# inai17ibar/video-diffusion-pipeline-parallel

Measured on AMD Instinct MI355X. Metric: steady-state videos/sec (whole node), SVD 14f x 25step, higher is better.
Workload: dtype f16

## Files before the change

video-diffusion-pipeline-parallel_amd/csrc/attention_long.hip:

```cpp
#include "common.h"

namespace {

typedef unsigned u32x4 __attribute__((ext_vector_type(4)));
typedef unsigned u32x2 __attribute__((ext_vector_type(2)));

__device__ __forceinline__ float fast_exp2(float x) { return __builtin_amdgcn_exp2f(x); }

constexpr unsigned LONG_BAIL_MIN = 64, LONG_BAIL_MAX = 512;

template <int QB>
__global__ __launch_bounds__(256, 1) void attn_long_kernel(
    const f16 *__restrict__ q, const f16 *__restrict__ k, const f16 *__restrict__ v, f16 *__restrict__ o,
    int64_t ldq, int64_t ldk, int64_t ldv, int64_t ldo, int seq, int heads, float scale_log2e,
    unsigned *__restrict__ flags) {
  constexpr int KV = 64;
  constexpr int K_BYTES = KV * 128, STAGE = 2 * K_BYTES, RING = 3;
  constexpr int OWN = 2 * QB;
  constexpr int WARM = OWN + 1;
  __shared__ __attribute__((aligned(16))) char smem[RING * STAGE];

  const int tid = threadIdx.x, lane = tid & 63;
  const int wave = __builtin_amdgcn_readfirstlane(tid >> 6);
  const int bh = blockIdx.y;
  {
    unsigned *const flagged_waves = flags + (int64_t)gridDim.x * gridDim.y;
    if (tid == 0) *(volatile unsigned *)smem = __hip_atomic_load(flagged_waves, __ATOMIC_RELAXED, __HIP_MEMORY_SCOPE_AGENT);
    __syncthreads();
    const unsigned seen = *(volatile unsigned *)smem;
    __syncthreads();
    const unsigned total_waves = gridDim.x * gridDim.y * 4u;
    const unsigned frac = total_waves / 16u;
    const unsigned bail = frac < LONG_BAIL_MIN ? LONG_BAIL_MIN : (frac > LONG_BAIL_MAX ? LONG_BAIL_MAX : frac);
    if (seen >= bail) {
      if (tid == 0) flags[(int64_t)bh * gridDim.x + blockIdx.x] = 1u;
      return;
    }
  }
  const int b = bh / heads, hd = bh - b * heads;
  const int r = lane & 31, h = lane >> 5;
  const int64_t row0 = (int64_t)b * seq;
  const int q0 = blockIdx.x * (128 * QB) + wave * (32 * QB);

  f16x8 qf[QB][4];
#pragma unroll
  for (int qb = 0; qb < QB; ++qb) {
    const f16 *qp = q + (row0 + q0 + qb * 32 + r) * ldq + hd * 64 + 8 * h;
#pragma unroll
    for (int s = 0; s < 4; ++s) {
      const f16x8 raw = *(const f16x8 *)(qp + 16 * s);
#pragma unroll
      for (int e = 0; e < 8; ++e) qf[qb][s][e] = (f16)((float)raw[e] * scale_log2e);
    }
  }

  const int lrow = lane >> 3, lchunk = lane & 7;
  unsigned kofl[2], vofl[2];
#pragma unroll
  for (int i = 0; i < 2; ++i) {
    const int row = wave * 16 + i * 8 + lrow;
    kofl[i] = (unsigned)((row * ldk + ((lchunk ^ ((row >> 1) & 7)) << 3)) * 2);
    vofl[i] = (unsigned)((row * ldv + ((lchunk ^ (((row >> 1) & 1) << 2)) << 3)) * 2);
  }
  const int64_t kstep = (int64_t)KV * ldk * 2, vstep = (int64_t)KV * ldv * 2;

  int koff[2];
#pragma unroll
  for (int kt = 0; kt < 2; ++kt) koff[kt] = (kt * 32 + r) * 128;
  int kswz = (r >> 1) & 7, hq = h;
  const int g = lane >> 4, i16 = lane & 15, q_ = i16 >> 2, pp = i16 & 3;
  const int vrow_l = 4 * (g >> 1) + q_;
  const int vchunk_l = 2 * (g & 1) + (pp >> 1);
  const int vswz = (q_ >> 1) << 2;
  const int vbyte_l = (pp & 1) * 8;
  int vlane0 = vrow_l * 128 + ((vchunk_l ^ vswz) << 4) + vbyte_l;
  int vlane1 = vrow_l * 128 + (((4 + vchunk_l) ^ vswz) << 4) + vbyte_l;

  f16x8 lsel;
  {
    const int m16 = lane & 15, kb4 = lane >> 4;
    const bool one = ((m16 & 7) == 0 && (kb4 & 1) == 0) || ((m16 & 7) == 4 && (kb4 & 1) == 1);
#pragma unroll
    for (int e = 0; e < 8; ++e) lsel[e] = one ? (f16)1.f : (f16)0.f;
  }

  f32x16 oacc[QB][2], negm[QB];
  f32x4 lacc[QB];
  float m_run[QB];
#pragma unroll
  for (int qb = 0; qb < QB; ++qb) {
    m_run[qb] = 0.f;
    lacc[qb] = (f32x4){0.f, 0.f, 0.f, 0.f};
#pragma unroll
    for (int e = 0; e < 16; ++e) { oacc[qb][0][e] = 0.f; oacc[qb][1][e] = 0.f; negm[qb][e] = 0.f; }
  }
  const int ntiles = seq / KV;

  const int own0 = blockIdx.x * OWN;
  const char *kbase = (const char *)(k + row0 * ldk + hd * 64);
  const char *vbase = (const char *)(v + row0 * ldv + hd * 64);
  auto stage = [&](int i, int buf) {
    const int tl = i < OWN ? own0 + i : (i - OWN < own0 ? i - OWN : i);
    const char *kb = kbase + tl * kstep, *vb = vbase + tl * vstep;
    char *sk = smem + buf * STAGE;
    char *sv = sk + K_BYTES;
#pragma unroll
    for (int j = 0; j < 2; ++j) {
      glds16(kb + kofl[j], sk + (wave * 16 + j * 8) * 128);
      glds16(vb + vofl[j], sv + (wave * 16 + j * 8) * 128);
    }
  };
  stage(0, 0);
  stage(1, 1);
  asm volatile("s_waitcnt vmcnt(4)" ::: "memory");
  __builtin_amdgcn_s_barrier();

  auto qk = [&](int qb, const char *sk, f32x16 (&sacc)[2]) {
    f16x8 kf[2][4];
#pragma unroll
    for (int kt = 0; kt < 2; ++kt)
#pragma unroll
      for (int s = 0; s < 4; ++s) kf[kt][s] = *(const f16x8 *)(sk + koff[kt] + (((2 * s + hq) ^ kswz) << 4));
#pragma unroll
    for (int kt = 0; kt < 2; ++kt)
#pragma unroll
      for (int s = 0; s < 4; ++s)
        sacc[kt] = __builtin_amdgcn_mfma_f32_32x32x16_f16(kf[kt][s], qf[qb][s], s == 0 ? negm[qb] : sacc[kt], 0, 0, 0);
  };
  auto pv = [&](int qb, const u32x4 (&pw)[2][2], const u32x2 (&vr)[2][8]) {
#pragma unroll
    for (int dt = 0; dt < 2; ++dt)
#pragma unroll
      for (int kt = 0; kt < 2; ++kt)
#pragma unroll
        for (int s = 0; s < 2; ++s) {
          const u32x4 vw = {vr[dt][4 * kt + 2 * s][0], vr[dt][4 * kt + 2 * s][1], vr[dt][4 * kt + 2 * s + 1][0],
                            vr[dt][4 * kt + 2 * s + 1][1]};
          oacc[qb][dt] = __builtin_amdgcn_mfma_f32_32x32x16_f16(__builtin_bit_cast(f16x8, vw),
                                                               __builtin_bit_cast(f16x8, pw[kt][s]), oacc[qb][dt], 0, 0, 0);
          if (dt == 0)
            lacc[qb] = __builtin_amdgcn_mfma_f32_16x16x32_f16(lsel, __builtin_bit_cast(f16x8, pw[kt][s]), lacc[qb], 0, 0, 0);
        }
  };

  auto warm_tile = [&](int i, int buf) {
    if (i + 2 < ntiles) stage(i + 2, buf >= 1 ? buf - 1 : RING - 1);
    const char *sk = smem + buf * STAGE;
    const char *sv = sk + K_BYTES;

    f32x16 sacc[2][2];
    u32x4 pw[2][2][2];
    qk(0, sk, sacc[0]);
    u32x2 vr[2][8];
    {
      const unsigned va[2] = {(unsigned)(uintptr_t)(const __attribute__((address_space(3))) char *)(sv + vlane0),
                              (unsigned)(uintptr_t)(const __attribute__((address_space(3))) char *)(sv + vlane1)};
#pragma unroll
      for (int dt = 0; dt < 2; ++dt)
#pragma unroll
        for (int j = 0; j < 8; ++j)
          asm volatile("ds_read_b64_tr_b16 %0, %1 offset:%2" : "=v"(vr[dt][j]) : "v"(va[dt]), "n"(j * 8 * 128) : "memory");
      asm volatile("s_waitcnt lgkmcnt(0)"
                   : "+v"(vr[0][0]), "+v"(vr[0][1]), "+v"(vr[0][2]), "+v"(vr[0][3]), "+v"(vr[0][4]), "+v"(vr[0][5]),
                     "+v"(vr[0][6]), "+v"(vr[0][7]), "+v"(vr[1][0]), "+v"(vr[1][1]), "+v"(vr[1][2]), "+v"(vr[1][3]),
                     "+v"(vr[1][4]), "+v"(vr[1][5]), "+v"(vr[1][6]), "+v"(vr[1][7])::"memory");
    }

#pragma unroll
    for (int qb = 0; qb < QB; ++qb) {
      f32x16(&sc)[2] = sacc[qb & 1];
      if (qb > 0) pv(qb - 1, pw[(qb - 1) & 1], vr);
      {
        float mt = fmaxf(fmaxf(sc[0][0], sc[0][1]), sc[0][2]);
#pragma unroll
        for (int e = 3; e < 31; e += 2) mt = fmaxf(fmaxf(mt, sc[e >> 4][e & 15]), sc[(e + 1) >> 4][(e + 1) & 15]);
        mt = fmaxf(mt, sc[1][15]);
        float ma = mt, mb = mt;
        asm volatile("s_nop 1\n\tv_permlane32_swap_b32 %0, %1" : "+v"(ma), "+v"(mb));
        mt = fmaxf(ma, mb);
        const float delta = i == 0 ? mt : fmaxf(mt, 0.f);
        if (__builtin_amdgcn_ballot_w64(delta != 0.f) != 0) {
          const float alpha = i == 0 ? 1.f : fast_exp2(-delta);
          lacc[qb][0] *= alpha;
#pragma unroll
          for (int e = 0; e < 16; ++e) { oacc[qb][0][e] *= alpha; oacc[qb][1][e] *= alpha; }
#pragma unroll
          for (int kt = 0; kt < 2; ++kt)
#pragma unroll
            for (int e = 0; e < 16; ++e) sc[kt][e] -= delta;
          m_run[qb] += delta;
#pragma unroll
          for (int e = 0; e < 16; ++e) negm[qb][e] = -m_run[qb];
        }
      }
      if (qb + 1 < QB) qk(qb + 1, sk, sacc[(qb + 1) & 1]);
      u32x4(&pc)[2][2] = pw[qb & 1];
#pragma unroll
      for (int kt = 0; kt < 2; ++kt)
#pragma unroll
        for (int e = 0; e < 16; e += 2) {
          const f32x2 p = {fast_exp2(sc[kt][e]), fast_exp2(sc[kt][e + 1])};
          pc[kt][e >> 3][(e & 7) >> 1] = __builtin_bit_cast(unsigned, __builtin_convertvector(p, f16x2));
        }
    }
    pv(QB - 1, pw[(QB - 1) & 1], vr);
    if (i + 2 < ntiles) asm volatile("s_waitcnt vmcnt(4)" ::: "memory"); else asm volatile("s_waitcnt vmcnt(0)" ::: "memory");
    __builtin_amdgcn_s_barrier();
  };

#ifdef LONG_TRACE
  unsigned tr[16] = {0}, tprev = (unsigned)__builtin_amdgcn_s_memtime();
#endif
  f16x8 kf[2][4];
  auto read_k = [&](int buf) {
    const char *sk = smem + buf * STAGE;
#pragma unroll
    for (int kt = 0; kt < 2; ++kt)
#pragma unroll
      for (int s = 0; s < 4; ++s) kf[kt][s] = *(const f16x8 *)(sk + koff[kt] + (((2 * s + hq) ^ kswz) << 4));
  };
  const char *kb2 = nullptr, *vb2 = nullptr;
  int tl2 = 0, o_cur = 0, o_nxt = 0, o_prv = 0;
  unsigned va[2] = {0u, 0u};
  const int kstep32 = (int)kstep, vstep32 = (int)vstep;
  auto lds_addr = [&](int off) { return (unsigned)(uintptr_t)(const __attribute__((address_space(3))) char *)(smem + off); };
  auto steady_setup = [&](int i, int buf) {
    const int vis = i + 2 < ntiles ? i + 2 : ntiles - 1;
    tl2 = vis < OWN ? own0 + vis : (vis - OWN < own0 ? vis - OWN : vis);
    kb2 = kbase + tl2 * kstep; vb2 = vbase + tl2 * vstep;
    o_cur = buf * STAGE;
    o_nxt = (buf + 1 == RING ? 0 : buf + 1) * STAGE;
    o_prv = (buf >= 1 ? buf - 1 : RING - 1) * STAGE;
    va[0] = lds_addr(o_cur + K_BYTES) + vlane0; va[1] = lds_addr(o_cur + K_BYTES) + vlane1;
  };
  auto steady2 = [&](int i) {
    static_assert(QB == 2, "the written-out schedule is for two query blocks");
    char *sk2 = smem + o_prv;
    auto dma = [&](int j, bool v_piece) {
      if (v_piece) glds16(vb2 + vofl[j], sk2 + K_BYTES + (wave * 16 + j * 8) * 128);
      else glds16(kb2 + kofl[j], sk2 + (wave * 16 + j * 8) * 128);
    };
    auto advance_global = [&]() {
      const int visn = i + 3 < ntiles ? i + 3 : ntiles - 1;
      const int tln = visn - OWN < own0 ? visn - OWN : visn;
      const int d = tln - tl2;
      kb2 += (unsigned)(d * kstep32); vb2 += (unsigned)(d * vstep32);
      tl2 = tln;
    };
    auto advance_slots = [&]() {
      const int t = o_prv; o_prv = o_cur; o_cur = o_nxt; o_nxt = t;
      va[0] = lds_addr(o_cur + K_BYTES) + vlane0; va[1] = lds_addr(o_cur + K_BYTES) + vlane1;
    };
    f32x16 sc[2][2];
    unsigned pw[2][2][2][4];
    u32x2 vr[2][8];
    auto S = [&](int b, int kt, int s) {
      sc[b][kt] = __builtin_amdgcn_mfma_f32_32x32x16_f16(kf[kt][s], qf[b][s], s == 0 ? negm[b] : sc[b][kt], 0, 0, 0);
    };
    auto Q = [&](int b, int kt, int s, int q) {
      const int e = 8 * s + 2 * q;
      const f32x2 p = {fast_exp2(sc[b][kt][e]), fast_exp2(sc[b][kt][e + 1])};
      pw[b][kt][s][q] = __builtin_bit_cast(unsigned, __builtin_convertvector(p, f16x2));
      asm volatile("" : "+v"(pw[b][kt][s][q]));
    };
    auto P = [&](int b, int kt, int s, int which) {
      const u32x4 pk = {pw[b][kt][s][0], pw[b][kt][s][1], pw[b][kt][s][2], pw[b][kt][s][3]};
      if (which == 1) {
        lacc[b] = __builtin_amdgcn_mfma_f32_16x16x32_f16(lsel, __builtin_bit_cast(f16x8, pk), lacc[b], 0, 0, 0);
      } else {
        const int dt = which >> 1;
        const u32x4 vw = {vr[dt][4 * kt + 2 * s][0], vr[dt][4 * kt + 2 * s][1], vr[dt][4 * kt + 2 * s + 1][0],
                          vr[dt][4 * kt + 2 * s + 1][1]};
        oacc[b][dt] = __builtin_amdgcn_mfma_f32_32x32x16_f16(__builtin_bit_cast(f16x8, vw), __builtin_bit_cast(f16x8, pk),
                                                            oacc[b][dt], 0, 0, 0);
      }
    };
#define SB() __builtin_amdgcn_sched_barrier(0)
#ifdef LONG_TRACE_ROWS
#define STAMP(k) { const unsigned t_ = (unsigned)__builtin_amdgcn_s_memtime(); tr[k] += t_ - tprev; tprev = t_; SB(); }
    STAMP(0);
#else
#define STAMP(k)
#endif
    auto RV = [&](int j) {
#pragma unroll
      for (int dt = 0; dt < 2; ++dt)
        asm volatile("ds_read_b64_tr_b16 %0, %1 offset:%2" : "=v"(vr[dt][j]) : "v"(va[dt]), "n"(j * 8 * 128) : "memory");
    };
    const char *skn = smem + o_nxt;
    auto RK = [&](int n) { kf[n >> 2][n & 3] = *(const f16x8 *)(skn + koff[n >> 2] + (((2 * (n & 3) + hq) ^ kswz) << 4)); };
#pragma unroll
    for (int s = 0; s < 4; ++s) { S(0, 0, s); SB(); }
    dma(0, false); SB();
    STAMP(1);
#pragma unroll
    for (int s = 0; s < 4; ++s) { S(0, 1, s); Q(0, 0, 0, s); SB(); }
#pragma unroll
    for (int s = 0; s < 4; ++s) { S(1, 0, s); Q(0, 0, 1, s); SB(); }
    dma(0, true); SB();
    STAMP(2);
#pragma unroll
    for (int s = 0; s < 4; ++s) { S(1, 1, s); Q(0, 1, 0, s); RV(s); SB(); }
    asm volatile("s_waitcnt lgkmcnt(0)"
                 : "+v"(vr[0][0]), "+v"(vr[0][1]), "+v"(vr[0][2]), "+v"(vr[0][3]), "+v"(vr[1][0]), "+v"(vr[1][1]), "+v"(vr[1][2]),
                   "+v"(vr[1][3])::"memory");
    SB();
    STAMP(3);
    P(0, 0, 0, 0); Q(0, 1, 1, 0); RV(4); SB();
    P(0, 0, 0, 1); Q(0, 1, 1, 1); RV(5); SB();
    P(0, 0, 0, 2); Q(0, 1, 1, 2); RV(6); SB();
    P(0, 0, 1, 0); Q(0, 1, 1, 3); RV(7); SB();
    P(0, 0, 1, 1); SB();
    P(0, 0, 1, 2); SB();
    asm volatile("s_waitcnt lgkmcnt(0)"
                 : "+v"(vr[0][4]), "+v"(vr[0][5]), "+v"(vr[0][6]), "+v"(vr[0][7]), "+v"(vr[1][4]), "+v"(vr[1][5]), "+v"(vr[1][6]),
                   "+v"(vr[1][7])::"memory");
    SB();
    STAMP(4);
    asm volatile("s_waitcnt vmcnt(2)" ::: "memory");
    __builtin_amdgcn_s_barrier();
    SB();
    STAMP(5);
#define ROW(pb, pkt, ps, qkt, qs, X0, X1, X2)                              \
    P(pb, pkt, ps, 0); Q(1, qkt, qs, 0); Q(1, qkt, qs, 1); X0; SB();       \
    P(pb, pkt, ps, 1); Q(1, qkt, qs, 2); X1; SB();                         \
    P(pb, pkt, ps, 2); Q(1, qkt, qs, 3); X2; SB();
    ROW(0, 1, 0, 0, 0, dma(1, false), , )
    ROW(0, 1, 1, 0, 1, dma(1, true), , )
    STAMP(6);
    ROW(1, 0, 0, 1, 0, RK(0), RK(1), RK(2))
    ROW(1, 0, 1, 1, 1, RK(3), RK(4), RK(5))
#undef ROW
    STAMP(7);
    P(1, 1, 0, 0); RK(6); SB();
    P(1, 1, 0, 1); RK(7); SB();
    P(1, 1, 0, 2); advance_global(); SB();
    P(1, 1, 1, 0); SB();
    P(1, 1, 1, 1); advance_slots(); SB();
    P(1, 1, 1, 2); SB();
    STAMP(8);
#undef SB
#undef STAMP
  };

  int buf = 0;
  for (int i = 0; i < WARM; ++i) {
    warm_tile(i, buf);
    buf = buf + 1 == RING ? 0 : buf + 1;
  }
#pragma unroll
  for (int qb = 0; qb < QB; ++qb)
#pragma unroll
    for (int s = 0; s < 4; ++s) asm volatile("" : "+v"(qf[qb][s]));
  asm volatile("" : "+v"(koff[0]), "+v"(koff[1]), "+v"(vlane0), "+v"(vlane1), "+v"(kofl[0]), "+v"(kofl[1]), "+v"(vofl[0]),
               "+v"(vofl[1]), "+v"(lsel), "+v"(kswz), "+v"(hq));
  read_k(buf);
#ifdef LONG_TRACE
  const unsigned long long tc0 = __builtin_amdgcn_s_memtime(), tw0 = wall_clock64();
#endif
  steady_setup(WARM, buf);
  for (int i = WARM; i < ntiles; ++i) steady2(i);
  asm volatile("s_waitcnt vmcnt(0)" ::: "memory");

#ifdef LONG_TRACE
  tr[14] = (unsigned)(__builtin_amdgcn_s_memtime() - tc0);
  tr[15] = (unsigned)(wall_clock64() - tw0);
  if (blockIdx.x == 3 && blockIdx.y == LONG_TRACE && tid < 16) flags[gridDim.x * gridDim.y + 1 + tid] = tr[tid];
#endif
  {
    bool bad = false;
#pragma unroll
    for (int qb = 0; qb < QB; ++qb) bad = bad || !(lacc[qb][0] < 3.0e38f);
    if (__builtin_amdgcn_ballot_w64(bad) != 0 && lane == 0) {
      flags[(int64_t)bh * gridDim.x + blockIdx.x] = 1u;
      __hip_atomic_fetch_add(flags + (int64_t)gridDim.x * gridDim.y, 1u, __ATOMIC_RELAXED, __HIP_MEMORY_SCOPE_AGENT);
    }
  }

#pragma unroll
  for (int qb = 0; qb < QB; ++qb) {
    const float inv = 1.0f / lacc[qb][0];
    f16 *op = o + (row0 + q0 + qb * 32 + r) * ldo + hd * 64 + 4 * h;
#pragma unroll
    for (int dt = 0; dt < 2; ++dt)
#pragma unroll
      for (int c = 0; c < 4; ++c) {
        f16x4 w;
#pragma unroll
        for (int e = 0; e < 4; ++e) w[e] = (f16)(oacc[qb][dt][4 * c + e] * inv);
        *(f16x4 *)(op + 32 * dt + 8 * c) = w;
      }
  }
}

}

constexpr int LONG_QB = 2;
constexpr int LONG_ROWS = 128 * LONG_QB;

int sp_attn_spatial_launch(const void *q, const void *k, const void *v, void *o, int64_t ldq, int64_t ldk, int64_t ldv,
                           int64_t ldo, int batch, int seq, int heads, float scale, const void *zero_page,
                           const unsigned *only_flagged, void *stream, const char *who);

extern "C" int64_t sp_attn_long_ws_bytes(int batch, int seq, int heads) {
  if (batch <= 0 || seq <= 0 || heads <= 0) return 0;
  return ((int64_t)batch * heads * ((seq + LONG_ROWS - 1) / LONG_ROWS) + 1) * (int64_t)sizeof(unsigned);
}

extern "C" int sp_attn_spatial_long_f16(const void *q, const void *k, const void *v, void *o, int64_t ldq, int64_t ldk,
                                        int64_t ldv, int64_t ldo, int batch, int seq, int heads, float scale,
                                        const void *zero_page, void *workspace, int64_t workspace_bytes, void *stream) {
  SP_REQUIRE(q && k && v && o && zero_page, "sp_attn_spatial_long_f16: null pointer");
  SP_REQUIRE(batch > 0 && seq > 0 && heads > 0, "sp_attn_spatial_long_f16: batch/seq/heads must be positive");
  if (!(seq >= 4096 && seq % LONG_ROWS == 0))
    return sp_attn_spatial_launch(q, k, v, o, ldq, ldk, ldv, ldo, batch, seq, heads, scale, zero_page, nullptr, stream,
                                  "sp_attn_spatial_long_f16");
  SP_REQUIRE(ldq % 8 == 0 && ldk % 8 == 0 && ldv % 8 == 0 && ldo % 4 == 0,
             "sp_attn_spatial_long_f16: strides must be multiples of 8");
  SP_REQUIRE((int64_t)batch * heads <= 65535, "sp_attn_spatial_long_f16: batch*heads too large");
  const int64_t need = sp_attn_long_ws_bytes(batch, seq, heads);
  SP_REQUIRE(workspace && ((uintptr_t)workspace & 3) == 0 && workspace_bytes >= need,
             "sp_attn_spatial_long_f16: workspace of %lld bytes, need %lld (4-byte aligned)", (long long)workspace_bytes,
             (long long)need);
  SP_REQUIRE(5 * 64 * ldk * 2 < (1ll << 31) && 5 * 64 * ldv * 2 < (1ll << 31), "sp_attn_spatial_long_f16: row stride too large");
  hipStream_t s = (hipStream_t)stream;
  unsigned *flags = (unsigned *)workspace;
  if (hipMemsetAsync(flags, 0, (size_t)need, s) != hipSuccess) {
    (void)hipGetLastError();
    sp_set_error("sp_attn_spatial_long_f16: hipMemsetAsync of the flag words failed");
    return SP_ELAUNCH;
  }
  SP_CLEAR_STALE_ERROR();
  hipLaunchKernelGGL(attn_long_kernel<LONG_QB>, dim3(seq / LONG_ROWS, batch * heads), dim3(256), 0, s, (const f16 *)q,
                     (const f16 *)k, (const f16 *)v, (f16 *)o, ldq, ldk, ldv, ldo, seq, heads, scale * 1.4426950408889634f,
                     flags);
  SP_CHECK_LAUNCH("sp_attn_spatial_long_f16");
  return sp_attn_spatial_launch(q, k, v, o, ldq, ldk, ldv, ldo, batch, seq, heads, scale, zero_page, flags, stream,
                                "sp_attn_spatial_long_f16(second pass)");
}
```

Measured before the change: 0.8214.

## Software-pipeline long attention across tile periods with prologue/epilogue peeling

Restructures the steady-state loop of the long-sequence attention kernel so that each period overlaps the PV MFMAs of the previous tile with the QK MFMAs of the current one, interleaving exp/convert, LDS reads and DMA issue at a finer granularity. First and last periods are peeled to handle the pipeline fill and drain, and score and probability registers now live across iterations. The intent is to hide softmax and LDS latency behind matrix work. The cost is higher register pressure and a wait count (vmcnt 4 instead of 2) that is more delicate to get right.

```diff
diff --git a/video-diffusion-pipeline-parallel_amd/csrc/attention_long.hip b/video-diffusion-pipeline-parallel_amd/csrc/attention_long.hip
--- a/video-diffusion-pipeline-parallel_amd/csrc/attention_long.hip
+++ b/video-diffusion-pipeline-parallel_amd/csrc/attention_long.hip
@@ -212,12 +212,10 @@
   unsigned tr[16] = {0}, tprev = (unsigned)__builtin_amdgcn_s_memtime();
 #endif
   f16x8 kf[2][4];
-  auto read_k = [&](int buf) {
+  auto read_k0 = [&](int buf) {
     const char *sk = smem + buf * STAGE;
 #pragma unroll
-    for (int kt = 0; kt < 2; ++kt)
-#pragma unroll
-      for (int s = 0; s < 4; ++s) kf[kt][s] = *(const f16x8 *)(sk + koff[kt] + (((2 * s + hq) ^ kswz) << 4));
+    for (int s = 0; s < 4; ++s) kf[0][s] = *(const f16x8 *)(sk + koff[0] + (((2 * s + hq) ^ kswz) << 4));
   };
   const char *kb2 = nullptr, *vb2 = nullptr;
   int tl2 = 0, o_cur = 0, o_nxt = 0, o_prv = 0;
@@ -233,10 +231,13 @@
     o_prv = (buf >= 1 ? buf - 1 : RING - 1) * STAGE;
     va[0] = lds_addr(o_cur + K_BYTES) + vlane0; va[1] = lds_addr(o_cur + K_BYTES) + vlane1;
   };
-  auto steady2 = [&](int i) {
+  f32x16 sc[2][2];
+  unsigned pw[2][2][2][4];
+  u32x2 vr[2][8];
+  auto period = [&](int i, const bool first, const bool last) __attribute__((always_inline)) {
     static_assert(QB == 2, "the written-out schedule is for two query blocks");
-    char *sk2 = smem + o_prv;
     auto dma = [&](int j, bool v_piece) {
+      char *sk2 = smem + o_prv;
       if (v_piece) glds16(vb2 + vofl[j], sk2 + K_BYTES + (wave * 16 + j * 8) * 128);
       else glds16(kb2 + kofl[j], sk2 + (wave * 16 + j * 8) * 128);
     };
@@ -251,10 +252,7 @@
       const int t = o_prv; o_prv = o_cur; o_cur = o_nxt; o_nxt = t;
       va[0] = lds_addr(o_cur + K_BYTES) + vlane0; va[1] = lds_addr(o_cur + K_BYTES) + vlane1;
     };
-    f32x16 sc[2][2];
-    unsigned pw[2][2][2][4];
-    u32x2 vr[2][8];
-    auto S = [&](int b, int kt, int s) {
+    auto S =[&](int b, int kt, int s) {
       sc[b][kt] = __builtin_amdgcn_mfma_f32_32x32x16_f16(kf[kt][s], qf[b][s], s == 0 ? negm[b] : sc[b][kt], 0, 0, 0);
     };
     auto Q = [&](int b, int kt, int s, int q) {
@@ -287,58 +285,59 @@
       for (int dt = 0; dt < 2; ++dt)
         asm volatile("ds_read_b64_tr_b16 %0, %1 offset:%2" : "=v"(vr[dt][j]) : "v"(va[dt]), "n"(j * 8 * 128) : "memory");
     };
-    const char *skn = smem + o_nxt;
-    auto RK = [&](int n) { kf[n >> 2][n & 3] = *(const f16x8 *)(skn + koff[n >> 2] + (((2 * (n & 3) + hq) ^ kswz) << 4)); };
-#pragma unroll
-    for (int s = 0; s < 4; ++s) { S(0, 0, s); SB(); }
-    dma(0, false); SB();
+    auto RK = [&](int n) {
+      kf[n >> 2][n & 3] = *(const f16x8 *)(smem + o_cur + koff[n >> 2] + (((2 * (n & 3) + hq) ^ kswz) << 4));
+    };
+#define WAIT_V(j0)                                                                                                          \
+    asm volatile("s_waitcnt lgkmcnt(0)"                                                                                     \
+                 : "+v"(vr[0][j0]), "+v"(vr[0][j0 + 1]), "+v"(vr[0][j0 + 2]), "+v"(vr[0][j0 + 3]), "+v"(vr[1][j0]),         \
+                   "+v"(vr[1][j0 + 1]), "+v"(vr[1][j0 + 2]), "+v"(vr[1][j0 + 3])::"memory");                                \
+    SB();
+#define PROW(on, pb, pkt, qb, qkt, X0, X1, X2, X3, X4)                     \
+    if (on) { P(pb, pkt, 0, 0); SB(); } X0; SB(); Q(qb, qkt, 0, 0); SB();  \
+    if (on) { P(pb, pkt, 0, 1); SB(); } X1; SB();                          \
+    if (on) { P(pb, pkt, 0, 2); SB(); } Q(qb, qkt, 0, 1); X2; SB();        \
+    if (on) { P(pb, pkt, 1, 0); SB(); } Q(qb, qkt, 0, 2); X3; SB();        \
+    if (on) { P(pb, pkt, 1, 1); SB(); } X4; SB();                          \
+    if (on) { P(pb, pkt, 1, 2); SB(); } Q(qb, qkt, 0, 3); SB();
+#define SROW(on, sb, skt, qb, qkt, X1)                                     \
+    if (on) { S(sb, skt, 0); SB(); } Q(qb, qkt, 1, 0); SB();               \
+    if (on) { S(sb, skt, 1); SB(); } Q(qb, qkt, 1, 1); X1; SB();           \
+    if (on) { S(sb, skt, 2); SB(); } Q(qb, qkt, 1, 2); SB();               \
+    if (on) { S(sb, skt, 3); SB(); } Q(qb, qkt, 1, 3); SB();
+    if (first) {
+#pragma unroll
+      for (int s = 0; s < 4; ++s) { S(0, 0, s); SB(); }
+    }
+    PROW(!first, 1, 1, 0, 0, RV(0), RV(1), RV(2), RV(3), if (first) dma(0, false))
+    WAIT_V(0)
     STAMP(1);
-#pragma unroll
-    for (int s = 0; s < 4; ++s) { S(0, 1, s); Q(0, 0, 0, s); SB(); }
-#pragma unroll
-    for (int s = 0; s < 4; ++s) { S(1, 0, s); Q(0, 0, 1, s); SB(); }
-    dma(0, true); SB();
+    SROW(true, 1, 0, 0, 0, dma(1, false))
     STAMP(2);
-#pragma unroll
-    for (int s = 0; s < 4; ++s) { S(1, 1, s); Q(0, 1, 0, s); RV(s); SB(); }
-    asm volatile("s_waitcnt lgkmcnt(0)"
-                 : "+v"(vr[0][0]), "+v"(vr[0][1]), "+v"(vr[0][2]), "+v"(vr[0][3]), "+v"(vr[1][0]), "+v"(vr[1][1]), "+v"(vr[1][2]),
-                   "+v"(vr[1][3])::"memory");
-    SB();
+    PROW(true, 0, 0, 1, 0, RK(4), RK(5), RK(6), RK(7), if (first) dma(0, true))
     STAMP(3);
-    P(0, 0, 0, 0); Q(0, 1, 1, 0); RV(4); SB();
-    P(0, 0, 0, 1); Q(0, 1, 1, 1); RV(5); SB();
-    P(0, 0, 0, 2); Q(0, 1, 1, 2); RV(6); SB();
-    P(0, 0, 1, 0); Q(0, 1, 1, 3); RV(7); SB();
-    P(0, 0, 1, 1); SB();
-    P(0, 0, 1, 2); SB();
-    asm volatile("s_waitcnt lgkmcnt(0)"
-                 : "+v"(vr[0][4]), "+v"(vr[0][5]), "+v"(vr[0][6]), "+v"(vr[0][7]), "+v"(vr[1][4]), "+v"(vr[1][5]), "+v"(vr[1][6]),
-                   "+v"(vr[1][7])::"memory");
-    SB();
+    SROW(true, 0, 1, 1, 0, dma(1, true))
     STAMP(4);
-    asm volatile("s_waitcnt vmcnt(2)" ::: "memory");
+    PROW(true, 1, 0, 0, 1, RV(4), RV(5), RV(6), RV(7), { advance_global(); advance_slots(); })
+    WAIT_V(4)
+    STAMP(5);
+    asm volatile("s_waitcnt vmcnt(4)" ::: "memory");
     __builtin_amdgcn_s_barrier();
     SB();
-    STAMP(5);
-#define ROW(pb, pkt, ps, qkt, qs, X0, X1, X2)                              \
-    P(pb, pkt, ps, 0); Q(1, qkt, qs, 0); Q(1, qkt, qs, 1); X0; SB();       \
-    P(pb, pkt, ps, 1); Q(1, qkt, qs, 2); X1; SB();                         \
-    P(pb, pkt, ps, 2); Q(1, qkt, qs, 3); X2; SB();
-    ROW(0, 1, 0, 0, 0, dma(1, false), , )
-    ROW(0, 1, 1, 0, 1, dma(1, true), , )
     STAMP(6);
-    ROW(1, 0, 0, 1, 0, RK(0), RK(1), RK(2))
-    ROW(1, 0, 1, 1, 1, RK(3), RK(4), RK(5))
-#undef ROW
+    SROW(true, 1, 1, 0, 1, dma(0, false))
     STAMP(7);
-    P(1, 1, 0, 0); RK(6); SB();
-    P(1, 1, 0, 1); RK(7); SB();
-    P(1, 1, 0, 2); advance_global(); SB();
-    P(1, 1, 1, 0); SB();
-    P(1, 1, 1, 1); advance_slots(); SB();
-    P(1, 1, 1, 2); SB();
+    PROW(true, 0, 1, 1, 1, if (!last) RK(0), if (!last) RK(1), if (!last) RK(2), if (!last) RK(3), )
     STAMP(8);
+    SROW(!last, 0, 0, 1, 1, dma(0, true))
+    STAMP(9);
+    if (last) {
+      P(1, 1, 0, 0); SB(); P(1, 1, 0, 1); SB(); P(1, 1, 0, 2); SB();
+      P(1, 1, 1, 0); SB(); P(1, 1, 1, 1); SB(); P(1, 1, 1, 2); SB();
+    }
+#undef PROW
+#undef SROW
+#undef WAIT_V
 #undef SB
 #undef STAMP
   };
@@ -354,12 +353,14 @@
     for (int s = 0; s < 4; ++s) asm volatile("" : "+v"(qf[qb][s]));
   asm volatile("" : "+v"(koff[0]), "+v"(koff[1]), "+v"(vlane0), "+v"(vlane1), "+v"(kofl[0]), "+v"(kofl[1]), "+v"(vofl[0]),
                "+v"(vofl[1]), "+v"(lsel), "+v"(kswz), "+v"(hq));
-  read_k(buf);
+  read_k0(buf);
 #ifdef LONG_TRACE
   const unsigned long long tc0 = __builtin_amdgcn_s_memtime(), tw0 = wall_clock64();
 #endif
   steady_setup(WARM, buf);
-  for (int i = WARM; i < ntiles; ++i) steady2(i);
+  period(WARM, true, false);
+  for (int i = WARM + 1; i < ntiles - 1; ++i) period(i, false, false);
+  period(ntiles - 1, false, true);
   asm volatile("s_waitcnt vmcnt(0)" ::: "memory");
 
 #ifdef LONG_TRACE
```

Result: no change. 0.8289 (median of 6 runs) (+0.9%).
